# leok7v/sqz

Hardware: AMD Instinct MI355X
Metric: encode MB/s + decode MB/s, 32KB window, batched blocks, 1/2/4/8 MI355X (higher is better)
Workload: dtype u8; 1 GPU; 4096 x 262144 B Zipf(s=1) byte blocks, window 2^15, one independent stream per block (BASELINE.json configs[2]); total_blocks=4096, blocks_per_gpu=4096, block_bytes=262144, win_bits=15, parallelism=1 rank; the N>1 runs shard this same batch (strong scaling), finder=index, device=AMD Radeon Graphics (gfx950:sramecc+:xnack-)

## Files before the change

### sqz_amd/csrc/huffman_emit.hip

```cpp
#define SQZ_SEC_TIMERS
#define SQZ_CHANGED_INLINING __forceinline__
#define SQZ_INSERT_INLINING __forceinline__
#include "sqz_tree.h"
#include "sqz_kernels.h"

namespace sqzk {

constexpr int kPendBits = 58;

struct EmitLds {
    TreeLds  tree;
    uint32_t code[kCodeSlots];
};


struct BitQueue {
    EmitLds* lds;
    uint8_t* out;
    uint64_t capacity;
    uint64_t bytes;
    uint64_t carry_v;
    int      carry;
    int      error;
    uint64_t pend_v;
// ... 142 lines not shown
    if ((t & kTokMatch) == 0) { return t <= 0xFFu; }
    const uint32_t len = (t >> 16) & 0x7FFFu, dist = t & 0xFFFFu;
    return len >= (uint32_t)kLenMin && len <= (uint32_t)kLenMax && dist >= 1u && dist <= 0x7FFFu;
}

template <bool kStats>
__global__ __launch_bounds__(kWave, kStats ? 1 : 4)
void huffman_emit_kernel(const uint32_t* __restrict__ tokens,
                         const uint64_t* __restrict__ tok_off,
                         const uint32_t* __restrict__ tok_count,
                         uint8_t* __restrict__ out,
                         const uint64_t* __restrict__ out_off,
                         uint64_t* __restrict__ out_bytes,
                         int32_t* __restrict__ err_out,
                         uint32_t n_blocks,
                         uint64_t prefix_acc, int prefix_fill,
                         sqz_block_stats* __restrict__ stats_out) {
    __shared__ EmitLds lds;
    const int lane = threadIdx.x;
    const uint32_t b = blockIdx.x;
    if (b >= n_blocks) { return; }

    using LitTree = LitTreeT<true, kStats>;
    using PosTree = PosTreeT<true, kStats>;
    LitTree lit; PosTree pos;
    lit.lds = &lds.tree; lit.code = lds.code; lit.lut = nullptr;
    pos.lds = &lds.tree; pos.code = lds.code; pos.lut = nullptr;
    lit.init_all(lane);
    pos.init_all(lane);
    for (int k = lane; k < kCodeSlots; k += kWave) { lds.code[k] = 0; }
    __syncthreads();

    const uint32_t* tok = tokens + uni64(tok_off[b]);
    uint32_t count = (uint32_t)__builtin_amdgcn_readfirstlane((int)tok_count[b]);
    const bool too_many = (uint64_t)count > uni64(tok_off[b + 1]) - uni64(tok_off[b]);
    if (too_many) { count = 0; }

    BitQueue q;
    q.lds = &lds;
    const uint64_t o0 = uni64(out_off[b]), o1 = uni64(out_off[b + 1]);
    q.out = out + o0;
    q.capacity = o1 - o0;
    q.bytes = 0;
    q.pend_v = 0;
    q.pend_n = 0;
    q.carry = prefix_fill;
    q.carry_v = prefix_fill > 0 ? (prefix_acc << (64 - prefix_fill)) : 0ull;
    q.error = 0;
    int err = 0;

    if (too_many) { err = kEINVAL; }
    if (!lit.insert_wave(kLitNyt, lane)) { err = kEINVAL; }
    if (!pos.insert_wave(kPosBase + kPosNyt, lane)) { err = kEINVAL; }

    uint32_t cursor = 0;
    uint32_t lit_tokens = 0, match_bytes = 0;
    uint32_t win0 = (uint32_t)lane < count ? tok[lane] : 0u;
    uint32_t win1 = (uint32_t)lane + (uint32_t)kWave < count ? tok[kWave + lane] : 0u;
#ifdef SQZ_STATS
    uint64_t es[4] = {0, 0, 0, 0}, es_last = __builtin_readcyclecounter(), es_begin = es_last;
    uint32_t es_steps = 0, es_exact = 0;
#define ES(k) { const uint64_t n_ = __builtin_readcyclecounter(); es[k] += n_ - es_last; es_last = n_; }
#else
#define ES(k)
#endif
    const uint32_t quarter = (count >> 2) + 1;
    int prio_now = -1;
    int want = 16, avg4 = 32;
    uint32_t regain_at = 0;
    while (cursor < count && err == 0) {
        {
            const int qq = (int)(cursor / quarter);
            if (qq != prio_now) {
                prio_now = qq;
                if (qq == 0) { __builtin_amdgcn_s_setprio(3); }
                else if (qq == 1) { __builtin_amdgcn_s_setprio(2); }
                else if (qq == 2) { __builtin_amdgcn_s_setprio(1); }
                else { __builtin_amdgcn_s_setprio(0); }
            }
        }
        const uint32_t step_start = cursor;
        const bool valid = cursor + (uint32_t)lane < count;
        const uint32_t traw = win0;
        const bool wellformed = token_ok(traw);
        const uint32_t t = wellformed ? traw : 0u;
        const bool is_match = (t & kTokMatch) != 0;
        Code lc = {0, 0, 0}, pc = {0, 0, 0};
        int a = (int)(t & 0xFFu), bsym = -1;
        uint32_t tlen = 1;
        if (is_match) {
            tlen = (t >> 16) & 0x1FFu;
            lc = len_code((int)tlen);
            pc = pos_code((int)(t & 0x7FFFu));
            a = kSymLen0 + lc.code;
            bsym = kPosBase + pc.code;
        }
        const bool new_a = valid && l_up(lds.tree.lnk[a]) == kNil;
        const bool new_b = valid && is_match && l_up(lds.tree.lnk[bsym]) == kNil;
        const uint64_t unseen = __ballot(valid && (new_a || new_b || !wellformed));
        const uint64_t vmask = __ballot(valid);
        int m = unseen != 0 ? __builtin_ctzll(unseen) : __builtin_popcountll(vmask);
        m = m < want ? m : want;
        if (cursor > kBatchTokens && (lit.aux | pos.aux) != 0) {
            lit.give_up_aux(lane);
            pos.give_up_aux(lane);
        }
        if ((lit.aux & pos.aux) == 0 && cursor <= kBatchTokens && cursor >= regain_at) {
            regain_at = cursor + 512u;
            (void)lit.regain_aux(lane);
            (void)pos.regain_aux(lane);
        }
        const bool frozen = (lit.complete | pos.complete) != 0 || lit.depth >= kFreezeDepth || pos.depth >= kFreezeDepth ||
                            (lit.aux & pos.aux) == 0;
        uint32_t ca = 0, cb = 0;
        int wa = 0, wb = 0;
        const int offered = m;
        ES(0)
        if (m >= 1 && !frozen) { m = bump_batch<true>(&lds.tree, lds.code, lit, pos, lane, m, a, bsym, ca, wa, cb, wb); }
        else { m = 0; }
        ES(1)
        if (m >= 1) {
            uint64_t v1 = ca, v2 = 0;
            uint32_t n1 = (uint32_t)wa, n2 = 0;
            if (is_match) {
                v1 = (v1 << lc.xbits) | (uint64_t)(lc.xbits ? (__brev((uint32_t)lc.extra) >> (32 - lc.xbits)) : 0u);
                n1 += (uint32_t)lc.xbits;
                v2 = ((uint64_t)cb << pc.xbits) | (uint64_t)(pc.xbits ? (__brev((uint32_t)pc.extra) >> (32 - pc.xbits)) : 0u);
                n2 = (uint32_t)(wb + pc.xbits);
            }
            if (lane >= m) { n1 = 0; n2 = 0; }
            q.pack_lanes(v1, n1, v2, n2, lane);
            if (kStats) {
                const uint64_t mm = __ballot(lane < m && is_match);
                lit_tokens += (uint32_t)(m - __builtin_popcountll(mm));
                match_bytes += wave_sum((lane < m && is_match) ? tlen : 0u);
            }
            cursor += (uint32_t)m;
        }
        ES(2)
        if (m < offered || offered == 0 || frozen) {
            const uint32_t tx = (uint32_t)__builtin_amdgcn_readlane((int)traw, m);
            if (!token_ok(tx)) { err = kEINVAL; break; }
            emit_token(q, lit, pos, tx, lane, err);
            if (kStats) { if ((tx & kTokMatch) != 0) { match_bytes += (tx >> 16) & 0x1FFu; } else { lit_tokens += 1; } }
            cursor += 1;
#ifdef SQZ_STATS
            es_exact++;
#endif
        }
        ES(3)
#ifdef SQZ_EMU_DEBUG_BATCH
        if (lane == 0) {
            static unsigned dbg_steps = 0, dbg_offered = 0, dbg_applied = 0, dbg_exact = 0, dbg_next = 16384;
            dbg_steps++; dbg_offered += (unsigned)offered; dbg_applied += (unsigned)m; dbg_exact += (m < offered || offered == 0 || frozen) ? 1u : 0u;
            if (cursor >= dbg_next || cursor >= count) {
                fprintf(stderr, "cursor %u: steps %u offered %u applied %u exact %u (want %d) depth %d/%d aux %d/%d\n", cursor, dbg_steps, dbg_offered, dbg_applied, dbg_exact, want,
                        lit.depth, pos.depth, lit.aux, pos.aux);
                dbg_steps = dbg_offered = dbg_applied = dbg_exact = 0; dbg_next = cursor + 16384;
            }
        }
#endif
#ifdef SQZ_STATS
        es_steps++;
#endif
        {
            avg4 += (int)(cursor - step_start) - (avg4 >> 2);
            want = ((avg4 * 3) >> 3) + 6;
            want = want < kWave ? want : kWave;
        }
        {
            const uint32_t adv = cursor - step_start;
            const int from = ((lane + (int)adv) & (kWave - 1)) * 4;
            const uint32_t s0 = (uint32_t)__builtin_amdgcn_ds_bpermute(from, (int)win0);
            const uint32_t s1 = (uint32_t)__builtin_amdgcn_ds_bpermute(from, (int)win1);
            win0 = (uint32_t)lane + adv < (uint32_t)kWave ? s0 : s1;
            const uint32_t t1 = cursor + (uint32_t)kWave + (uint32_t)lane;
            win1 = t1 < count ? tok[t1] : 0u;
        }
        if (q.error != 0) { err = q.error; }
        if (lit.fault | pos.fault) { err = kE2BIG; }
    }

#ifdef SQZ_STATS
    if (lane == 0 && b == 1) {
        printf("emit block 1: cycles %llu steps %u exact %u: prep %llu bump %llu pack %llu exact %llu\n",
               (unsigned long long)(es_last - es_begin), es_steps, es_exact, (unsigned long long)es[0],
               (unsigned long long)es[1], (unsigned long long)es[2], (unsigned long long)es[3]);
        for (int k = 0; k < 32; k++) { if (g_secn[k]) { printf("sec %d: %llu cycles / %u = %llu\n", k, g_sec[k], g_secn[k], g_sec[k] / g_secn[k]); } }
        printf("emit slow: lit insert %u/%llu changed %u/%llu; pos insert %u/%llu changed %u/%llu\n",
               lit.st_cnt[0], (unsigned long long)lit.st_cyc[0], lit.st_cnt[1], (unsigned long long)lit.st_cyc[1],
               pos.st_cnt[0], (unsigned long long)pos.st_cyc[0], pos.st_cnt[1], (unsigned long long)pos.st_cyc[1]);
    }
#endif
    if (err == 0) { q.flush(lane); err = q.error; }
    else { q.pack(lane); }
    if (lane == 0) {
        out_bytes[b] = q.bytes;
        err_out[b] = err;
        if (kStats && stats_out != nullptr) {
            sqz_block_stats* st = stats_out + b;
            st->lit_updates = lit.stats.updates; st->lit_swaps = lit.stats.swaps; st->lit_moves = lit.stats.moves;
            st->pos_updates = pos.stats.updates; st->pos_swaps = pos.stats.swaps; st->pos_moves = pos.stats.moves;
            st->literal_bytes = lit_tokens; st->backref_bytes = match_bytes;
            st->lit_depth = (uint32_t)lit.depth; st->pos_depth = (uint32_t)pos.depth;
            st->tokens = cursor; st->reserved = 0;
        }
    }
    if (kStats && stats_out != nullptr) {
        for (int k = lane; k < kLitLeaves; k += kWave) { stats_out[b].lit_freq[k] = lit.freq(k); }
        if (lane < kPosLeaves) { stats_out[b].pos_freq[lane] = pos.freq(kPosBase + lane); }
    }
}

using DbgLit = LitTreeT<true, true>;
using DbgPos = PosTreeT<true, true>;
template <class T>
__device__ __forceinline__ void debug_drive(T& t, DbgLit& lit, DbgPos& pos, EmitLds& lds, const int32_t* symbols,
                                            uint32_t count, int batch, int lane, bool is_pos, bool stop_early,
                                            uint32_t max_steps, uint32_t& consumed) {
    uint32_t k = 0;
    for (uint32_t step = 0; k < count && t.fault == 0 && (max_steps == 0 || step < max_steps); step++) {
        if (stop_early && t.aux == 0) { break; }
        int sym = -1;
        if (k + (uint32_t)lane < count) { sym = symbols[k + lane]; }
        const bool valid = sym >= 0 && sym < T::kLeaves && lane < batch;
        const int leaf = valid ? T::kBase + sym : T::kRoot;
        const uint64_t seen = __ballot(valid && l_up(lds.tree.lnk[leaf]) != kNil);
        int m = (~seen == 0ull) ? kWave : __builtin_ctzll(~seen);
        const bool frozen = t.complete != 0 || t.depth >= kFreezeDepth || t.aux == 0;
        uint32_t ca, cb; int wa, wb;
        if (m > 0 && !frozen) {
            m = is_pos ? bump_batch<true>(&lds.tree, lds.code, lit, pos, lane, m, -1, leaf, ca, wa, cb, wb)
                       : bump_batch<true>(&lds.tree, lds.code, lit, pos, lane, m, leaf, -1, ca, wa, cb, wb);
        } else { m = 0; }
        k += (uint32_t)m;
        if (k < count) {
            const int s = __builtin_amdgcn_readfirstlane(symbols[k]);
            if (s < 0 || s >= T::kLeaves) { break; }
            const int lf = T::kBase + s;
            const Chain c = t.chain_up(lf, lane);
            if (c.levels == 0) { (void)t.insert_wave(lf, lane); }
            else { (void)t.bump_wave(lf, c, lane); }
            k++;
        }
    }
    consumed = k;
}

__global__ __launch_bounds__(kWave, 4)
void tree_debug_kernel(const int32_t* __restrict__ symbols, uint32_t count, int which, int batch,
                       uint32_t* __restrict__ dump) {
    __shared__ EmitLds lds;
    const int lane = threadIdx.x;
    DbgLit lit; DbgPos pos;
    lit.lds = &lds.tree; lit.code = lds.code; lit.lut = nullptr;
    pos.lds = &lds.tree; pos.code = lds.code; pos.lut = nullptr;
    lit.init_all(lane);
    pos.init_all(lane);
    for (int k = lane; k < kCodeSlots; k += kWave) { lds.code[k] = 0; }
    __syncthreads();
    const bool stop_early = (batch & 0x100) != 0;
    batch &= 0xFF;
    if (batch < 1) { batch = 1; }
    if (batch > kWave) { batch = kWave; }
    const uint32_t max_steps = (uint32_t)which >> 8;
    which &= 1;
    uint32_t consumed = 0;
    if (which == 0) { debug_drive(lit, lit, pos, lds, symbols, count, batch, lane, false, stop_early, max_steps, consumed); }
    else { debug_drive(pos, lit, pos, lds, symbols, count, batch, lane, true, stop_early, max_steps, consumed); }
    lds_fence();
    const int base = which == 0 ? 0 : kPosBase, nodes = which == 0 ? kLitNodes : kPosNodes;
    const int leaves = which == 0 ? kLitLeaves : kPosLeaves, pos0 = which == 0 ? 0 : kPosPos0;
    if (lane == 0) {
        const TreeStats st = which == 0 ? lit.stats : pos.stats;
        dump[0] = (uint32_t)(which == 0 ? lit.next : pos.next);
        dump[1] = (uint32_t)(which == 0 ? lit.depth : pos.depth);
        dump[2] = (uint32_t)(which == 0 ? lit.complete : pos.complete);
        dump[3] = (uint32_t)(which == 0 ? lit.aux : pos.aux);
        dump[4] = (uint32_t)(which == 0 ? lit.fault : pos.fault) | (max_steps != 0 ? consumed << 8 : 0u);
        dump[5] = st.updates; dump[6] = st.swaps; dump[7] = st.moves;
    }
    for (int v = lane; v < nodes; v += kWave) {
        dump[8 + 4 * v + 0] = lds.tree.lnk[base + v];
        dump[8 + 4 * v + 1] = lds.tree.rng[base + v];
        dump[8 + 4 * v + 2] = lds.tree.cnt[base + v];
        dump[8 + 4 * v + 3] = v < leaves ? lds.code[pos0 + v] : 0u;
    }
}

void launch_tree_debug(const int32_t* symbols, uint32_t count, int which, int batch, uint32_t* dump,
                       hipStream_t stream) {
    hipLaunchKernelGGL(tree_debug_kernel, dim3(1), dim3(kWave), 0, stream, symbols, count, which, batch, dump);
}

void launch_huffman_emit(const uint32_t* tokens, const uint64_t* tok_off,
                         const uint32_t* tok_count, uint8_t* out,
                         const uint64_t* out_off, uint64_t* out_bytes,
                         int32_t* err, uint32_t n_blocks,
                         uint64_t prefix_acc, int prefix_fill, sqz_block_stats* stats,
                         hipStream_t stream) {
    if (n_blocks == 0) { return; }
    if (stats != nullptr) {
        hipLaunchKernelGGL(huffman_emit_kernel<true>, dim3(n_blocks), dim3(kWave), 0, stream,
                           tokens, tok_off, tok_count, out, out_off, out_bytes, err, n_blocks,
                           prefix_acc, prefix_fill, stats);
    } else {
        hipLaunchKernelGGL(huffman_emit_kernel<false>, dim3(n_blocks), dim3(kWave), 0, stream,
// ... 7 lines not shown
```

### sqz_amd/csrc/sqz_tree.h

```cpp
#pragma once

#include "sqz_device.h"

namespace sqzk {

constexpr uint32_t kNil = 0x3FFu;
constexpr int kLitLeaves = 288;
constexpr int kLitNodes  = kLitLeaves + 288;
constexpr int kPosLeaves = 32;
constexpr int kPosNodes  = 64;
constexpr int kPosBase   = kLitNodes;
constexpr int kAllNodes  = kLitNodes + kPosNodes;
constexpr int kPosPos0   = kLitLeaves;
constexpr int kPositions = kLitLeaves + kPosLeaves;
constexpr int kCodeSlots = kPositions;

constexpr uint32_t kCountMask = (1u << 24) - 1u;
constexpr int kDepthShift = 24;

#ifndef SQZ_AUX_DEPTH
#define SQZ_AUX_DEPTH 26
#endif
#ifndef SQZ_MAX_FAST_DEPTH
#define SQZ_MAX_FAST_DEPTH 60
#endif
#ifndef SQZ_FREEZE_DEPTH
#define SQZ_FREEZE_DEPTH 63
#endif
#ifndef SQZ_BATCH_TOKENS
#define SQZ_BATCH_TOKENS ((1u << 24) - 256u)
#endif
constexpr uint32_t kBatchTokens = SQZ_BATCH_TOKENS;
constexpr int kAuxDepth = SQZ_AUX_DEPTH;
constexpr int kMaxFastDepth = SQZ_MAX_FAST_DEPTH;
constexpr int kFreezeDepth = SQZ_FREEZE_DEPTH;
constexpr int kStack = 128;
constexpr int kTokenBits = 2 * (kAuxDepth - 1) + 18;
constexpr int kPackWords = (63 + 58 + kWave * kTokenBits + 63) / 64 + 1;
constexpr int kImageWords = kPackWords > kWave ? kPackWords : kWave;

#if defined(SQZ_STATS) && defined(SQZ_SEC_TIMERS)
__device__ unsigned long long g_sec[32];
__device__ unsigned int g_secn[32];
#define SEC_BEGIN uint64_t sec_t_ = __builtin_readcyclecounter();
#define SEC(k) { const uint64_t n_ = __builtin_readcyclecounter(); if (blockIdx.x == 1 && threadIdx.x == 0) { g_sec[k] += n_ - sec_t_; g_secn[k]++; } sec_t_ = n_; }
#define XSEC_BEGIN uint64_t xsec_t_ = __builtin_readcyclecounter();
#define XSEC(k) { const uint64_t n_ = __builtin_readcyclecounter(); if (blockIdx.x == 1 && threadIdx.x == 0) { g_sec[k] += n_ - xsec_t_; g_secn[k]++; } xsec_t_ = n_; }
#else
#define SEC_BEGIN
#define SEC(k)
#define XSEC_BEGIN
#define XSEC(k)
#endif

struct TreeLds {
    uint32_t lnk[kAllNodes];
    uint32_t rng[kAllNodes];
    uint32_t cnt[kAllNodes];
    uint32_t pend[kWave];
    uint16_t lvl[kStack];
    union { uint64_t P64[kImageWords]; uint32_t P32[2 * kImageWords]; uint8_t P8[8 * kImageWords]; };
};

struct TreeStats { uint32_t updates, swaps, moves; };

__device__ __forceinline__ void lds_fence() {
    __builtin_amdgcn_fence(__ATOMIC_SEQ_CST, "wavefront");
    asm volatile("" ::: "memory");
}

__device__ __forceinline__ uint32_t l_up(uint32_t w) { return w & 0x3FFu; }
__device__ __forceinline__ uint32_t l_lo(uint32_t w) { return (w >> 10) & 0x3FFu; }
__device__ __forceinline__ uint32_t l_hi(uint32_t w) { return (w >> 20) & 0x3FFu; }
__device__ __forceinline__ uint32_t mk_lnk(uint32_t up, uint32_t lo, uint32_t hi) { return up | (lo << 10) | (hi << 20); }
__device__ __forceinline__ uint32_t r_pos(uint32_t w) { return w & 0x1FFu; }
__device__ __forceinline__ uint32_t r_first(uint32_t w) { return w & 0x3FFu; }
__device__ __forceinline__ uint32_t r_last(uint32_t w) { return (w >> 10) & 0x3FFu; }
__device__ __forceinline__ uint32_t r_pa(uint32_t w) { return (w >> 20) & 0x3FFu; }
constexpr uint32_t kEndsMask = 0xFFFFFu;
constexpr uint32_t kNoPos = 0x1FFu;
__device__ __forceinline__ uint32_t c_f(uint32_t w) { return w & kCountMask; }
__device__ __forceinline__ uint32_t c_d(uint32_t w) { return (w >> kDepthShift) & 0x3Fu; }

__device__ __forceinline__ uint32_t wave_max(uint32_t v) {
    auto mx = [](uint32_t a, uint32_t b) { return a > b ? a : b; };
    v = mx(v, (uint32_t)__builtin_amdgcn_update_dpp(0, (int)v, 0x111 , 0xf, 0xf, false));
    v = mx(v, (uint32_t)__builtin_amdgcn_update_dpp(0, (int)v, 0x112 , 0xf, 0xf, false));
    v = mx(v, (uint32_t)__builtin_amdgcn_update_dpp(0, (int)v, 0x114 , 0xf, 0xf, false));
    v = mx(v, (uint32_t)__builtin_amdgcn_update_dpp(0, (int)v, 0x118 , 0xf, 0xf, false));
    v = mx(v, (uint32_t)__builtin_amdgcn_update_dpp(0, (int)v, 0x142 , 0xa, 0xf, false));
    v = mx(v, (uint32_t)__builtin_amdgcn_update_dpp(0, (int)v, 0x143 , 0xc, 0xf, false));
    return (uint32_t)__builtin_amdgcn_readlane((int)v, kWave - 1);
}

__device__ __forceinline__ uint32_t wave_sum(uint32_t v) {
    return (uint32_t)__builtin_amdgcn_readlane((int)wave_scan(v), kWave - 1);
}

struct Chain {
    int mine, par;
    int levels;
    bool holds;
    bool active;
    bool has_g;
};

#ifndef SQZ_INSERT_INLINING
#define SQZ_INSERT_INLINING __noinline__
#endif
#ifndef SQZ_LUT_INLINING
#define SQZ_LUT_INLINING __noinline__
#endif
template <class T> __device__ SQZ_INSERT_INLINING uint32_t slow_insert(TreeLds* lds, uint32_t* code, uint32_t regs, int sym, int lane);
#ifndef SQZ_CHANGED_INLINING
#define SQZ_CHANGED_INLINING __noinline__
#endif
template <class T> __device__ SQZ_CHANGED_INLINING uint32_t slow_changed(TreeLds* lds, uint32_t* code, uint32_t regs, int sym, int mine, int levels, int lane);
template <class T> __device__ SQZ_LUT_INLINING void slow_build_lut(const uint32_t* lnk, uint16_t* lut, int lane);

template <int BASE, int LEAVES, int NODES, int REF_LEAVES, int POS0, int LUT_BITS, bool CODES, bool STATS>
struct Tree {
    TreeLds* lds;
    uint32_t* code;
    uint16_t* lut;
    int next;
    int depth;
    int complete;
    int fault;
    int aux;
    int lut_ok;
    int in_insert;
    TreeStats stats;

    static constexpr int kBase = BASE;
    static constexpr int kRoot = BASE + LEAVES;
    static constexpr int kLeaves = LEAVES;
    static constexpr int kLutBits = LUT_BITS;
    static constexpr int kChgSlot = BASE == 0 ? 57 : 59;
    static constexpr int kIdEnd = BASE + ((LEAVES + 1 + REF_LEAVES - 2) < NODES ? (LEAVES + 1 + REF_LEAVES - 2) : NODES);
    static constexpr bool kCodes = CODES;
    static constexpr int kLeafRows = (LEAVES + kWave - 1) / kWave;

    __device__ __forceinline__ void init_all(int lane) {
        for (int i = BASE + lane; i < BASE + NODES; i += kWave) {
            lds->lnk[i] = 0x3FFFFFFFu;
            lds->rng[i] = kNoPos | (kNil << 20);
            lds->cnt[i] = 0;
        }
        next = kRoot + 1; depth = 0; complete = 0; fault = 0; aux = 1; lut_ok = 0; in_insert = 0;
        stats.updates = stats.swaps = stats.moves = 0;
    }

    __device__ __forceinline__ bool is_leaf(uint32_t v) const { return v < (uint32_t)kRoot; }
    __device__ __forceinline__ uint32_t up_of(int i) const { return l_up(lds->lnk[i]); }
    __device__ __forceinline__ uint32_t freq(int i) const { const uint32_t w = lds->cnt[i]; return aux != 0 ? c_f(w) : w; }
    __device__ __forceinline__ void set_freq(int i, uint32_t f) {
        lds->cnt[i] = aux != 0 ? ((lds->cnt[i] & ~kCountMask) | (f & kCountMask)) : f;
    }
    __device__ __forceinline__ int depth_by_walk(int v) const {
        int d = 0;
        for (uint32_t a = l_up(lds->lnk[v]); a != kNil && d < kStack; a = l_up(lds->lnk[a])) { d++; }
        return d;
    }
    __device__ __forceinline__ void give_up_aux(int lane) {
        if (aux == 0) { return; }
        aux = 0;
        for (int v = BASE + lane; v < BASE + NODES; v += kWave) { lds->cnt[v] &= kCountMask; }
        lds_fence();
    }
    __device__ __forceinline__ int code_slot(int leaf) const { return leaf - BASE + POS0; }
    __device__ __forceinline__ uint32_t first_leaf(uint32_t v) const { return is_leaf(v) ? v : r_first(lds->rng[v]); }
    __device__ __forceinline__ uint32_t last_leaf(uint32_t v) const { return is_leaf(v) ? v : r_last(lds->rng[v]); }
    __device__ __forceinline__ uint32_t pos_of(uint32_t leaf) const { return r_pos(lds->rng[leaf]); }
    __device__ __forceinline__ void set_ends(int v, uint32_t first, uint32_t last) {
        lds->rng[v] = (lds->rng[v] & ~kEndsMask) | first | (last << 10);
    }

    __device__ __forceinline__ uint32_t pack_regs() const {
        return (uint32_t)next | ((uint32_t)(depth & 0xFF) << 10) | ((uint32_t)(complete & 1) << 18) |
               ((uint32_t)(fault & 1) << 19) | ((uint32_t)(aux & 1) << 20);
    }
    __device__ __forceinline__ void unpack_regs(uint32_t r) {
        next = (int)(r & 0x3FFu); depth = (int)((r >> 10) & 0xFFu);
        complete = (int)((r >> 18) & 1u); fault = (int)((r >> 19) & 1u); aux = (int)((r >> 20) & 1u);
    }
    __device__ __forceinline__ void uniform_regs() {
        next = __builtin_amdgcn_readfirstlane(next);
        depth = __builtin_amdgcn_readfirstlane(depth);
        complete = __builtin_amdgcn_readfirstlane(complete);
        fault = __builtin_amdgcn_readfirstlane(fault);
        aux = __builtin_amdgcn_readfirstlane(aux);
    }
// ... 732 lines not shown
                                                           : mk_lnk(l_up(bw), l_lo(bw), (uint32_t)fresh);
                lds->lnk[at] = mk_lnk((uint32_t)fresh, kNil, kNil);
                lds->lnk[leaf] = mk_lnk((uint32_t)fresh, kNil, kNil);
                if (aux != 0) {
                    lds->cnt[at] = acw + (1u << kDepthShift);
                    lds->cnt[leaf] = 1u | ((c_d(acw) + 1u) << kDepthShift);
                    lds->rng[fresh] = (uint32_t)at | ((uint32_t)leaf << 10) | (kNil << 20);
                }
                sum(fresh);
                at = fresh;
            }
            hand = (uint32_t)leaf | ((uint32_t)at << 10) | (ok << 20) | (split << 21) | (q << 22);
        }
        uniform_regs();
        hand = (uint32_t)__builtin_amdgcn_readfirstlane((int)hand);
        lds_fence();
        int start = (int)(hand & 0x3FFu);
        const int at = (int)((hand >> 10) & 0x3FFu);
        const bool ok = ((hand >> 20) & 1u) != 0, split = ((hand >> 21) & 1u) != 0;
        const uint32_t q = hand >> 22;
        if (split && aux != 0) {
            const int fresh = at;
            const uint32_t leaf_at = l_lo(lds->lnk[fresh]);
            uint32_t ws[kLeafRows];
#pragma unroll
            for (int r = 0; r < kLeafRows; r++) {
                const int v = BASE + r * kWave + lane;
                ws[r] = lds->rng[v < kRoot ? v : kRoot];
            }
#pragma unroll
            for (int r = 0; r < kLeafRows; r++) {
                const int v = BASE + r * kWave + lane;
                if (BASE + r * kWave >= kRoot) { continue; }
                const uint32_t w = ws[r];
                if (v < kRoot && v != i && r_pos(w) != kNoPos && r_pos(w) > q) { lds->rng[v] = w + 1u; }
            }
            if (lane == 0) {
                lds->rng[i] = (q + 1u) | (kNil << 20);
                if (CODES) {
                    const uint32_t oc = code[code_slot((int)leaf_at)];
                    code[code_slot((int)leaf_at)] = oc << 1;
                    code[code_slot(i)] = (oc << 1) | 1u;
                }
            }
            lds_fence();
            fix_partners((int)l_up(lds->lnk[fresh]), 2, lane);
        }
        uint32_t droot = 0;
        if (!split && ok) {
            const uint32_t w = lds->lnk[at];
            if (__builtin_amdgcn_readfirstlane(
                    (l_lo(w) != kNil && l_hi(w) != kNil && freq((int)l_lo(w)) > freq((int)l_hi(w))) ? 1 : 0) != 0) {
                if (lane == 0) { lds->lnk[at] = mk_lnk(l_up(w), l_hi(w), l_lo(w)); }
                lds_fence();
                start = start == (int)l_lo(w) ? (int)l_hi(w) : (int)l_lo(w);
                swap_fix_at(at, droot, lane);
            }
        }
        if (depth + 4 >= kMaxFastDepth) {
            give_up_aux(lane);
            if (lane == 0) { changed(start); relabel(at); }
            uniform_regs();
            lds_fence();
        } else {
            const Chain c = chain_up(start, lane);
            in_insert = 1;
            changed_all(c, lane);
            if (aux != 0) { mark_subtree(at, lane); }
            else { if (lane == 0) { relabel(at); } uniform_regs(); lds_fence(); }
            in_insert = 0;
        }
        return ok;
    }
};

template <class T>
__device__ SQZ_INSERT_INLINING uint32_t slow_insert(TreeLds* lds, uint32_t* code, uint32_t regs, int sym, int lane) {
    T t;
    t.lds = lds; t.code = code; t.lut = nullptr; t.lut_ok = 0;
    t.stats.updates = t.stats.swaps = t.stats.moves = 0;
    t.unpack_regs(regs);
    const bool ok = t.insert_all(sym, lane);
    t.store_stats_delta(lane);
    return (uint32_t)__builtin_amdgcn_readfirstlane((int)(t.pack_regs() | (ok ? 0x80000000u : 0u)));
}

template <class T>
__device__ SQZ_CHANGED_INLINING uint32_t slow_changed(TreeLds* lds, uint32_t* code, uint32_t regs, int sym, int mine, int levels, int lane) {
    T t;
    t.lds = lds; t.code = code; t.lut = nullptr; t.lut_ok = 0;
    t.stats.updates = t.stats.swaps = t.stats.moves = 0;
    t.unpack_regs(regs);
    if (lane == 0) { t.lds->cnt[sym] += 1u; }
    lds_fence();
    if (t.depth + 4 >= kMaxFastDepth) {
        t.give_up_aux(lane);
        if (lane == 0) { t.changed(sym); }
        t.uniform_regs();
        lds_fence();
    } else {
        t.changed_all(t.make_chain(mine, levels, lane), lane);
    }
    t.store_stats_delta(lane);
    return (uint32_t)__builtin_amdgcn_readfirstlane((int)t.pack_regs());
}

template <class T>
__device__ __forceinline__ uint32_t lut_descend(const uint32_t* lnk, uint32_t parent, int bit, int level) {
    const uint32_t node = parent & 0x3FFu;
    const bool inside = node != kNil && node >= (uint32_t)T::kRoot;
    const uint32_t w = lnk[inside ? (int)node : (int)T::kRoot];
    const uint32_t child = bit ? l_hi(w) : l_lo(w);
    return inside ? (child | ((uint32_t)level << 10)) : parent;
}

template <class T>
__device__ SQZ_LUT_INLINING void slow_build_lut(const uint32_t* lnk, uint16_t* lut, int lane) {
    static_assert(T::kLutBits == 6 || T::kLutBits == 8, "table widths the decoder uses");
    const int half = (lane >> 1) * 4;
    const int bit = lane & 1;
    uint32_t e = (uint32_t)T::kRoot;
#pragma unroll
    for (int level = 1; level <= 6; level++) {
        const uint32_t parent = (uint32_t)__builtin_amdgcn_ds_bpermute(half, (int)e);
        e = lut_descend<T>(lnk, parent, bit, level);
    }
    if (T::kLutBits == 6) {
        lut[lane] = (uint16_t)e;
        return;
    }
    const uint32_t p0 = (uint32_t)__builtin_amdgcn_ds_bpermute(half, (int)e);
    const uint32_t p1 = (uint32_t)__builtin_amdgcn_ds_bpermute(half + 128, (int)e);
    const uint32_t r0 = lut_descend<T>(lnk, p0, bit, 7);
    const uint32_t r1 = lut_descend<T>(lnk, p1, bit, 7);
    const uint32_t q0 = (uint32_t)__builtin_amdgcn_ds_bpermute(half, (int)r0);
    const uint32_t q1 = (uint32_t)__builtin_amdgcn_ds_bpermute(half + 128, (int)r0);
    const uint32_t q2 = (uint32_t)__builtin_amdgcn_ds_bpermute(half, (int)r1);
    const uint32_t q3 = (uint32_t)__builtin_amdgcn_ds_bpermute(half + 128, (int)r1);
    lut[lane]       = (uint16_t)lut_descend<T>(lnk, q0, bit, 8);
    lut[lane + 64]  = (uint16_t)lut_descend<T>(lnk, q1, bit, 8);
    lut[lane + 128] = (uint16_t)lut_descend<T>(lnk, q2, bit, 8);
    lut[lane + 192] = (uint16_t)lut_descend<T>(lnk, q3, bit, 8);
}

template <bool CODES, bool STATS> using LitTreeT = Tree<0, kLitLeaves, kLitNodes, 512, 0, 8, CODES, STATS>;
template <bool CODES, bool STATS> using PosTreeT = Tree<kPosBase, kPosLeaves, kPosNodes, 32, kPosPos0, 6, CODES, STATS>;

template <bool kWantCode, class LIT, class POS>
__device__ __forceinline__ int bump_batch(TreeLds* lds, const uint32_t* code, const LIT& lit, const POS& pos,
                                          int lane, int m, int a, int b,
                                          uint32_t& code_a, int& depth_a, uint32_t& code_b, int& depth_b) {
    SEC_BEGIN
    const bool take = lane < m;
    const bool has_a = take && a >= 0, has_b = take && b >= 0;
    const int ia = has_a ? a : LIT::kRoot - 1, ib = has_b ? b : POS::kRoot - 1;
    constexpr int kLitRows = (kLitNodes - kLitLeaves + kWave - 1) / kWave;
    constexpr int kRows = kLitRows + 1;
    int vi[kRows];
    bool on[kRows];
#pragma unroll
    for (int row = 0; row < kLitRows; row++) {
        const int v = LIT::kRoot + row * kWave + lane;
        on[row] = v < lit.next && v != LIT::kRoot;
        vi[row] = on[row] ? v : LIT::kRoot;
    }
    {
        const int v = POS::kRoot + lane;
        on[kLitRows] = v < pos.next && v != POS::kRoot;
        vi[kLitRows] = on[kLitRows] ? v : POS::kRoot;
    }
    const uint32_t ra = lds->rng[ia], rb = lds->rng[ib];
    const uint32_t wa = lds->cnt[ia], wb = lds->cnt[ib];
    uint32_t rw[kRows], cw[kRows];
#pragma unroll
    for (int k = 0; k < kRows; k++) { rw[k] = lds->rng[vi[k]]; cw[k] = lds->cnt[vi[k]]; }
    if (kWantCode) {
        code_a = code[has_a ? ia - LIT::kBase + 0 : 0];
        code_b = code[has_b ? ib - POS::kBase + kPosPos0 : 0];
    }
    const uint32_t qa = r_pos(ra), qb = r_pos(rb);
    depth_a = (int)c_d(wa);
    depth_b = (int)c_d(wb);
    const uint32_t pa_a = r_pa(ra), pa_b = r_pa(rb);
    const uint32_t cpa = lds->cnt[pa_a != kNil ? pa_a : (uint32_t)ia], cpb = lds->cnt[pa_b != kNil ? pa_b : (uint32_t)ib];
    uint32_t cp[kRows], rf[kRows], rl[kRows];
#pragma unroll
    for (int k = 0; k < kRows; k++) {
        const uint32_t pk = r_pa(rw[k]);
        cp[k] = lds->cnt[pk != kNil ? pk : (uint32_t)vi[k]];
        rf[k] = lds->rng[r_first(rw[k])];
        rl[k] = lds->rng[r_last(rw[k])];
    }
    SEC(0)
    auto histogram = [&](int upto) {
        lds->P64[lane] = 0ull;
        lds_fence();
        if (lane < upto && has_a) { atomicAdd(&lds->P32[qa >> 2], 1u << (8u * (qa & 3u))); }
        if (lane < upto && has_b) { atomicAdd(&lds->P32[qb >> 2], 1u << (8u * (qb & 3u))); }
        lds_fence();
        const uint64_t h = lds->P64[lane];
        const uint64_t incl = h * 0x0101010101010101ull;
        const uint32_t total = (uint32_t)(incl >> 56);
        const uint32_t base = wave_scan(total) - total;
        lds->P64[lane] = (incl << 8) + (uint64_t)base * 0x0101010101010101ull;
        lds_fence();
    };
    histogram(m);
    SEC(1)
    uint32_t st[kRows], en[kRows], pst[kRows], pen[kRows];
#pragma unroll
    for (int k = 0; k < kRows; k++) { st[k] = r_pos(rf[k]); en[k] = r_pos(rl[k]) + 1u; }
    const uint32_t p_a0 = lds->P8[qa], p_a1 = lds->P8[qa + 1u], p_b0 = lds->P8[qb], p_b1 = lds->P8[qb + 1u];
#pragma unroll
    for (int k = 0; k < kRows; k++) { pst[k] = lds->P8[st[k]]; pen[k] = lds->P8[en[k]]; }
    auto pack = [](uint32_t s0, uint32_t e0, uint32_t f, uint32_t fb) {
        const uint32_t allowed = fb > f ? fb - f : 0u;
        return s0 | (e0 << 9) | ((allowed < 255u ? allowed : 255u) << 18);
    };
    uint32_t nl[kLitRows], sel[kLitRows], np = 0, sep = 0;
    uint32_t bad = 0;
    uint32_t sa, sb;
    {
        const uint32_t n = has_a ? p_a1 - p_a0 : 0u, f = c_f(wa), fb = c_f(cpa);
        sa = pack(qa, qa + 1u, f, fb);
        bad |= (n != 0 && pa_a != kNil && f + n > fb) ? 1u : 0u;
    }
    {
        const uint32_t n = has_b ? p_b1 - p_b0 : 0u, f = c_f(wb), fb = c_f(cpb);
        sb = pack(qb, qb + 1u, f, fb);
        bad |= (n != 0 && pa_b != kNil && f + n > fb) ? 2u : 0u;
    }
#pragma unroll
    for (int k = 0; k < kRows; k++) {
        const uint32_t n = on[k] ? pen[k] - pst[k] : 0u, f = c_f(cw[k]), fb = c_f(cp[k]);
        const uint32_t packed = on[k] ? pack(st[k], en[k], f, fb) : 0u;
        const bool fails = n != 0 && r_pa(rw[k]) != kNil && f + n > fb;
        if (k < kLitRows) { nl[k] = n; sel[k] = packed; bad |= fails ? (4u << k) : 0u; }
        else { np = n; sep = packed; bad |= fails ? 128u : 0u; }
    }
    int ok = m;
    SEC(2)
    if (__ballot(bad != 0) != 0) {
#pragma unroll
        for (int cat = 0; cat < 8; cat++) {
            uint64_t vm = __ballot((bad >> cat) & 1u);
            const uint32_t mine = cat == 0 ? sa : cat == 1 ? sb : cat == 7 ? sep : sel[cat >= 2 && cat < 7 ? cat - 2 : 0];
            while (vm != 0) {
                const int k = __builtin_ctzll(vm);
                vm &= vm - 1;
                const uint32_t t = (uint32_t)__builtin_amdgcn_readlane((int)mine, k);
                const uint32_t s0 = t & 0x1FFu, e0 = (t >> 9) & 0x1FFu, allowed = t >> 18;
                const bool through = (has_a && qa >= s0 && qa < e0) || (has_b && qb >= s0 && qb < e0);
                const uint64_t tm = __ballot(through);
                const uint64_t first_bad = __ballot(through && lanes_under(tm) == allowed);
                if (first_bad != 0) { const int j = __builtin_ctzll(first_bad); ok = j < ok ? j : ok; }
            }
        }
        if (ok == 0) { return 0; }
        histogram(ok);
#pragma unroll
        for (int row = 0; row < kLitRows; row++) {
            nl[row] = (uint32_t)lds->P8[(sel[row] >> 9) & 0x1FFu] - (uint32_t)lds->P8[sel[row] & 0x1FFu];
        }
        np = (uint32_t)lds->P8[(sep >> 9) & 0x1FFu] - (uint32_t)lds->P8[sep & 0x1FFu];
    }
    SEC(3)
    if (lane < ok && has_a) { atomicAdd(&lds->cnt[ia], 1u); }
    if (lane < ok && has_b) { atomicAdd(&lds->cnt[ib], 1u); }
#pragma unroll
    for (int row = 0; row < kLitRows; row++) {
        const int v = LIT::kRoot + row * kWave + lane;
        if (nl[row] != 0) { atomicAdd(&lds->cnt[v], nl[row]); }
    }
    if (np != 0) { atomicAdd(&lds->cnt[POS::kRoot + lane], np); }
    lds_fence();
    SEC(4)
    return ok;
}

}
```

Measured before the change: 15510 MB/s.

## Pack distance-tree internals into literal tree's last row and pre-cut batch at sibling-swap lanes

The batched Huffman weight bump now places the distance tree's internal nodes in the unused upper half of the literal tree's last wave row. This removes one row of LDS gathers, checks and atomics per batch. It also adds an early ballot that truncates the batch at the first lane whose leaf already has weight at least its parent's, so the slower per-category conflict scan runs less often. The early cut may shorten batches more than strictly needed, which means more steps overall.

```diff
diff --git a/sqz_amd/csrc/huffman_emit.hip b/sqz_amd/csrc/huffman_emit.hip
--- a/sqz_amd/csrc/huffman_emit.hip
+++ b/sqz_amd/csrc/huffman_emit.hip
@@ -318,7 +318,7 @@
 #ifdef SQZ_EMU_DEBUG_BATCH
         if (lane == 0) {
             static unsigned dbg_steps = 0, dbg_offered = 0, dbg_applied = 0, dbg_exact = 0, dbg_next = 16384;
-            dbg_steps++; dbg_offered += (unsigned)offered; dbg_applied += (unsigned)m; dbg_exact += (m < offered || offered == 0 || frozen) ? 1u : 0u;
+            dbg_steps++; dbg_offered += (unsigned)offered - g_dbg_cut; g_dbg_cut = 0; dbg_applied += (unsigned)m; dbg_exact += (m < offered || offered == 0 || frozen) ? 1u : 0u;
             if (cursor >= dbg_next || cursor >= count) {
                 fprintf(stderr, "cursor %u: steps %u offered %u applied %u exact %u (want %d) depth %d/%d aux %d/%d\n", cursor, dbg_steps, dbg_offered, dbg_applied, dbg_exact, want,
                         lit.depth, pos.depth, lit.aux, pos.aux);
diff --git a/sqz_amd/csrc/sqz_tree.h b/sqz_amd/csrc/sqz_tree.h
--- a/sqz_amd/csrc/sqz_tree.h
+++ b/sqz_amd/csrc/sqz_tree.h
@@ -38,6 +38,10 @@
 constexpr int kTokenBits = 2 * (kAuxDepth - 1) + 18;
 constexpr int kPackWords = (63 + 58 + kWave * kTokenBits + 63) / 64 + 1;
 constexpr int kImageWords = kPackWords > kWave ? kPackWords : kWave;
+
+#ifdef SQZ_EMU_DEBUG_BATCH
+static unsigned g_dbg_cut;
+#endif
 
 #if defined(SQZ_STATS) && defined(SQZ_SEC_TIMERS)
 __device__ unsigned long long g_sec[32];
@@ -1076,28 +1080,33 @@
                                           uint32_t& code_a, int& depth_a, uint32_t& code_b, int& depth_b) {
     SEC_BEGIN
     const bool take = lane < m;
-    const bool has_a = take && a >= 0, has_b = take && b >= 0;
+    bool has_a = take && a >= 0, has_b = take && b >= 0;
     const int ia = has_a ? a : LIT::kRoot - 1, ib = has_b ? b : POS::kRoot - 1;
-    constexpr int kLitRows = (kLitNodes - kLitLeaves + kWave - 1) / kWave;
-    constexpr int kRows = kLitRows + 1;
-    int vi[kRows];
-    bool on[kRows];
-#pragma unroll
-    for (int row = 0; row < kLitRows; row++) {
+    constexpr int kLitInner = kLitNodes - kLitLeaves, kPosInner = kPosNodes - kPosLeaves;
+    constexpr int kLitRows = (kLitInner + kWave - 1) / kWave;
+    constexpr int kLastRow = kLitRows - 1, kLastLit = kLastRow * kWave;
+    static_assert(kLitInner % kWave != 0 && kLitInner % kWave <= kWave / 2, "the literal tree leaves half of its last row free");
+    static_assert(kPosInner <= kWave / 2, "the distance tree's internal nodes fit that half row");
+    static_assert(kPosPos0 >= kLitLeaves, "the leaf positions of the two trees do not overlap");
+    int vi[kLitRows];
+    bool on[kLitRows];
+#pragma unroll
+    for (int row = 0; row < kLastRow; row++) {
         const int v = LIT::kRoot + row * kWave + lane;
         on[row] = v < lit.next && v != LIT::kRoot;
         vi[row] = on[row] ? v : LIT::kRoot;
     }
     {
-        const int v = POS::kRoot + lane;
-        on[kLitRows] = v < pos.next && v != POS::kRoot;
-        vi[kLitRows] = on[kLitRows] ? v : POS::kRoot;
+        const bool in_pos = lane >= kWave / 2;
+        const int v = in_pos ? POS::kRoot + lane - kWave / 2 : LIT::kRoot + kLastLit + lane;
+        on[kLastRow] = in_pos ? (v < pos.next && v != POS::kRoot) : v < lit.next;
+        vi[kLastRow] = on[kLastRow] ? v : (in_pos ? POS::kRoot : LIT::kRoot);
     }
     const uint32_t ra = lds->rng[ia], rb = lds->rng[ib];
     const uint32_t wa = lds->cnt[ia], wb = lds->cnt[ib];
-    uint32_t rw[kRows], cw[kRows];
-#pragma unroll
-    for (int k = 0; k < kRows; k++) { rw[k] = lds->rng[vi[k]]; cw[k] = lds->cnt[vi[k]]; }
+    uint32_t rw[kLitRows], cw[kLitRows];
+#pragma unroll
+    for (int k = 0; k < kLitRows; k++) { rw[k] = lds->rng[vi[k]]; cw[k] = lds->cnt[vi[k]]; }
     if (kWantCode) {
         code_a = code[has_a ? ia - LIT::kBase + 0 : 0];
         code_b = code[has_b ? ib - POS::kBase + kPosPos0 : 0];
@@ -1107,18 +1116,20 @@
     depth_b = (int)c_d(wb);
     const uint32_t pa_a = r_pa(ra), pa_b = r_pa(rb);
     const uint32_t cpa = lds->cnt[pa_a != kNil ? pa_a : (uint32_t)ia], cpb = lds->cnt[pa_b != kNil ? pa_b : (uint32_t)ib];
-    uint32_t cp[kRows], rf[kRows], rl[kRows];
-#pragma unroll
-    for (int k = 0; k < kRows; k++) {
+    uint32_t cp[kLitRows], rf[kLitRows], rl[kLitRows];
+#pragma unroll
+    for (int k = 0; k < kLitRows; k++) {
         const uint32_t pk = r_pa(rw[k]);
         cp[k] = lds->cnt[pk != kNil ? pk : (uint32_t)vi[k]];
         rf[k] = lds->rng[r_first(rw[k])];
         rl[k] = lds->rng[r_last(rw[k])];
     }
     SEC(0)
+    auto clear_histogram = [&]() {
+        lds->P64[lane] = 0ull;
+        lds_fence();
+    };
     auto histogram = [&](int upto) {
-        lds->P64[lane] = 0ull;
-        lds_fence();
         if (lane < upto && has_a) { atomicAdd(&lds->P32[qa >> 2], 1u << (8u * (qa & 3u))); }
         if (lane < upto && has_b) { atomicAdd(&lds->P32[qb >> 2], 1u << (8u * (qb & 3u))); }
         lds_fence();
@@ -1129,19 +1140,51 @@
         lds->P64[lane] = (incl << 8) + (uint64_t)base * 0x0101010101010101ull;
         lds_fence();
     };
+    clear_histogram();
+#ifdef SQZ_EMU_DEBUG_BATCH
+    const int dbg_m = m;
+    const uint64_t dbg_sa = __ballot(has_a && pa_a != kNil && c_f(cpa) <= c_f(wa));
+    const uint64_t dbg_sb = __ballot(has_b && pa_b != kNil && c_f(cpb) <= c_f(wb));
+    const uint64_t dbg_nil = __ballot((has_a && pa_a == kNil) || (has_b && pa_b == kNil));
+    uint64_t dbg_bad[2 + kLitRows] = {};
+    auto dbg_line = [&](int cut, int applied) {
+        if (lane != 0) { return; }
+        fprintf(stderr, "batch m %d cut %d a %llx b %llx nil %llx bad", dbg_m, cut, (unsigned long long)dbg_sa,
+                (unsigned long long)dbg_sb, (unsigned long long)dbg_nil);
+        for (int c = 0; c < 2 + kLitRows; c++) { fprintf(stderr, " %llx", (unsigned long long)dbg_bad[c]); }
+        fprintf(stderr, " ok %d next %d %d\n", applied, lit.next - LIT::kRoot, pos.next - POS::kRoot);
+    };
+#endif
+#ifndef SQZ_BATCH_NO_CUT
+    {
+        const uint64_t stops = __ballot((has_a && pa_a != kNil && c_f(cpa) <= c_f(wa)) ||
+                                        (has_b && pa_b != kNil && c_f(cpb) <= c_f(wb)));
+        if (stops != 0) {
+            const int j = __builtin_ctzll(stops);
+#ifdef SQZ_EMU_DEBUG_BATCH
+            if (lane == 0) { g_dbg_cut += (unsigned)(m - j); }
+            if (j == 0) { dbg_line(0, 0); }
+#endif
+            m = j;
+            if (m == 0) { return 0; }
+            has_a = has_a && lane < m;
+            has_b = has_b && lane < m;
+        }
+    }
+#endif
     histogram(m);
     SEC(1)
-    uint32_t st[kRows], en[kRows], pst[kRows], pen[kRows];
-#pragma unroll
-    for (int k = 0; k < kRows; k++) { st[k] = r_pos(rf[k]); en[k] = r_pos(rl[k]) + 1u; }
+    uint32_t st[kLitRows], en[kLitRows], pst[kLitRows], pen[kLitRows];
+#pragma unroll
+    for (int k = 0; k < kLitRows; k++) { st[k] = r_pos(rf[k]); en[k] = r_pos(rl[k]) + 1u; }
     const uint32_t p_a0 = lds->P8[qa], p_a1 = lds->P8[qa + 1u], p_b0 = lds->P8[qb], p_b1 = lds->P8[qb + 1u];
 #pragma unroll
-    for (int k = 0; k < kRows; k++) { pst[k] = lds->P8[st[k]]; pen[k] = lds->P8[en[k]]; }
+    for (int k = 0; k < kLitRows; k++) { pst[k] = lds->P8[st[k]]; pen[k] = lds->P8[en[k]]; }
     auto pack = [](uint32_t s0, uint32_t e0, uint32_t f, uint32_t fb) {
         const uint32_t allowed = fb > f ? fb - f : 0u;
         return s0 | (e0 << 9) | ((allowed < 255u ? allowed : 255u) << 18);
     };
-    uint32_t nl[kLitRows], sel[kLitRows], np = 0, sep = 0;
+    uint32_t nl[kLitRows], sel[kLitRows];
     uint32_t bad = 0;
     uint32_t sa, sb;
     {
@@ -1155,20 +1198,22 @@
         bad |= (n != 0 && pa_b != kNil && f + n > fb) ? 2u : 0u;
     }
 #pragma unroll
-    for (int k = 0; k < kRows; k++) {
+    for (int k = 0; k < kLitRows; k++) {
         const uint32_t n = on[k] ? pen[k] - pst[k] : 0u, f = c_f(cw[k]), fb = c_f(cp[k]);
-        const uint32_t packed = on[k] ? pack(st[k], en[k], f, fb) : 0u;
-        const bool fails = n != 0 && r_pa(rw[k]) != kNil && f + n > fb;
-        if (k < kLitRows) { nl[k] = n; sel[k] = packed; bad |= fails ? (4u << k) : 0u; }
-        else { np = n; sep = packed; bad |= fails ? 128u : 0u; }
+        nl[k] = n;
+        sel[k] = on[k] ? pack(st[k], en[k], f, fb) : 0u;
+        bad |= (n != 0 && r_pa(rw[k]) != kNil && f + n > fb) ? (4u << k) : 0u;
     }
     int ok = m;
     SEC(2)
+#ifdef SQZ_EMU_DEBUG_BATCH
+    for (int c = 0; c < 2 + kLitRows; c++) { dbg_bad[c] = __ballot((bad >> c) & 1u); }
+#endif
     if (__ballot(bad != 0) != 0) {
 #pragma unroll
-        for (int cat = 0; cat < 8; cat++) {
+        for (int cat = 0; cat < 2 + kLitRows; cat++) {
             uint64_t vm = __ballot((bad >> cat) & 1u);
-            const uint32_t mine = cat == 0 ? sa : cat == 1 ? sb : cat == 7 ? sep : sel[cat >= 2 && cat < 7 ? cat - 2 : 0];
+            const uint32_t mine = cat == 0 ? sa : cat == 1 ? sb : sel[cat >= 2 ? cat - 2 : 0];
             while (vm != 0) {
                 const int k = __builtin_ctzll(vm);
                 vm &= vm - 1;
@@ -1180,25 +1225,29 @@
                 if (first_bad != 0) { const int j = __builtin_ctzll(first_bad); ok = j < ok ? j : ok; }
             }
         }
+#ifdef SQZ_EMU_DEBUG_BATCH
+        if (ok == 0) { dbg_line(m < dbg_m ? m : -1, 0); }
+#endif
         if (ok == 0) { return 0; }
+        clear_histogram();
         histogram(ok);
 #pragma unroll
         for (int row = 0; row < kLitRows; row++) {
             nl[row] = (uint32_t)lds->P8[(sel[row] >> 9) & 0x1FFu] - (uint32_t)lds->P8[sel[row] & 0x1FFu];
         }
-        np = (uint32_t)lds->P8[(sep >> 9) & 0x1FFu] - (uint32_t)lds->P8[sep & 0x1FFu];
     }
     SEC(3)
     if (lane < ok && has_a) { atomicAdd(&lds->cnt[ia], 1u); }
     if (lane < ok && has_b) { atomicAdd(&lds->cnt[ib], 1u); }
 #pragma unroll
     for (int row = 0; row < kLitRows; row++) {
-        const int v = LIT::kRoot + row * kWave + lane;
-        if (nl[row] != 0) { atomicAdd(&lds->cnt[v], nl[row]); }
-    }
-    if (np != 0) { atomicAdd(&lds->cnt[POS::kRoot + lane], np); }
+        if (nl[row] != 0) { atomicAdd(&lds->cnt[vi[row]], nl[row]); }
+    }
     lds_fence();
     SEC(4)
+#ifdef SQZ_EMU_DEBUG_BATCH
+    dbg_line(m < dbg_m ? m : -1, ok);
+#endif
     return ok;
 }
 
```

Result: faster. 15870 MB/s, median of 6 (+2.3%).
